# AI-Unicamp/GestureDiffusion

Hardware: AMD Instinct MI355X
Metric: denoised motion frames/sec (1000-step p_sample_loop, B=64, T=196, d=512) (higher is better)
Workload: dtype f32; 1 GPU; BASELINE config 2: MDM_Old (V1 encoder-only topology) J=263 d=512 ff=1024 L=8 H=4, 1000-step p_sample_loop, batch 64/GPU x 196 frames, random weights, in-kernel Philox noise; global_batch=64, frames=196, parallelism=dp1 (independent samples, end-of-loop gather), step=one denoising step (forward + fused sampler update) over the rank's batch

## Files before the change

gesturediffusion_amd/_lib.py:

```python
import ctypes as C
import os

_HERE = os.path.dirname(os.path.abspath(__file__))
LIB_PATH = os.environ.get("GDX_LIBGDX") or os.path.join(_HERE, "csrc", "libgdx.so")

GDX_ARCH_MDM_OLD, GDX_ARCH_MDM = 1, 2
GDX_COND, GDX_UNCOND, GDX_CFG = 0, 1, 2
GDX_SAMPLER_P, GDX_SAMPLER_DDIM = 0, 1
GDX_ROW_PAD = 256

EXPORTS = [
    "gdx_create", "gdx_destroy", "gdx_last_error", "gdx_set_weight", "gdx_weights_ready", "gdx_prepare",
    "gdx_set_condition", "gdx_forward", "gdx_set_keep_taps", "gdx_get_tap", "gdx_sampler_update", "gdx_q_sample",
    "gdx_randn", "gdx_sample_loop", "gdx_bench_ffn_gemm", "gdx_bench_gemm", "gdx_forward_flops", "gdx_profile_begin", "gdx_profile_end", "gdx_bench_attention",
    "gdx_linear_f16", "gdx_linear_f32", "gdx_bench_gemm_f16", "gdx_attention_f16", "gdx_attention_f32", "gdx_plms_update", "gdx_postprocess", "gdx_q_sample_t", "gdx_masked_l2", "gdx_set_graph_replay", "gdx_mfcc",
    "gdx_set_guards", "gdx_check_guards", "gdx_packed_bytes", "gdx_export_packed", "gdx_import_packed", "gdx_set_test_half_dtype",
    "gdx_set_test_gemmh_tile", "gdx_linear_half", "gdx_layernorm", "gdx_local_attention", "gdx_attention_half",
    "gdx_bpd_terms", "gdx_bpd_loop", "gdx_linear_full", "gdx_plms_step", "gdx_plms_loop",
    "gdx_dpm_step", "gdx_dpm_loop", "gdx_dpm_sde_step", "gdx_dpm_sde_loop",
    "gdx_set_guidance_interval", "gdx_forward_samples", "gdx_set_guidance_rescale", "gdx_cfg_rescale",
    "gdx_transpose_in", "gdx_transpose_out", "gdx_small_linear", "gdx_gather_rows", "gdx_mfcc_project", "gdx_token0",
]
GDX_BPD_CHUNK = 4096
INT64_MIN, INT64_MAX = -2**63, 2**63 - 1


class GdxError(RuntimeError):
    pass


class Config(C.Structure):
    _fields_ = [(n, C.c_int32) for n in ("arch", "njoints", "latent_dim", "ff_size", "num_layers", "num_heads",
                                         "seed_poses", "mfcc_dim", "cl_head", "window", "compute_dtype")]


class UpdateArgs(C.Structure):
    _fields_ = [
        ("kind", C.c_int32), ("batch", C.c_int32), ("njoints", C.c_int32), ("frames", C.c_int32),
        ("coef", C.c_void_p), ("t", C.c_void_p), ("step_index", C.c_int32),
        ("x", C.c_void_p), ("x0_cond", C.c_void_p), ("x0_uncond", C.c_void_p), ("scale", C.c_void_p),
        ("inpaint_mask", C.c_void_p), ("inpaint_motion", C.c_void_p), ("noise", C.c_void_p),
        ("const_noise", C.c_int32), ("philox_seed", C.c_uint64), ("sample_offset", C.c_uint64),
        ("rng_step", C.c_uint32), ("out", C.c_void_p), ("pred_xstart", C.c_void_p),
        ("cond_grad", C.c_void_p), ("cond_coef", C.c_void_p), ("clip_denoised", C.c_int32),
    ]


class PlmsArgs(C.Structure):
    _fields_ = [
        ("kind", C.c_int32), ("batch", C.c_int32), ("per_sample", C.c_int64), ("coef", C.c_void_p), ("t", C.c_void_p),
        ("step_index", C.c_int32), ("x", C.c_void_p), ("pred_xstart", C.c_void_p), ("eps", C.c_void_p * 4),
        ("out", C.c_void_p),
    ]

# ... 108 lines not shown
                       f"(run `python __graft_entry__.py` or `make -C gesturediffusion_amd/csrc`)")
    try:
        import torch
        lib = C.CDLL(LIB_PATH)
    except OSError as e:
        raise GdxError(f"cannot load {LIB_PATH}: {e}") from e
    vp, i32, i64, u64, u32 = C.c_void_p, C.c_int32, C.c_int64, C.c_uint64, C.c_uint32
    lib.gdx_last_error.restype = C.c_char_p
    sigs = {
        "gdx_create": [C.POINTER(Config), C.POINTER(vp)],
        "gdx_destroy": [vp],
        "gdx_set_weight": [vp, C.c_char_p, vp, C.POINTER(i64), i32, vp],
        "gdx_weights_ready": [vp],
        "gdx_prepare": [vp, i32, i32],
        "gdx_set_condition": [vp, vp, vp, vp],
        "gdx_forward": [vp, vp, vp, i32, vp, vp, vp],
        "gdx_set_keep_taps": [vp, i32],
        "gdx_get_tap": [vp, i32, vp, i64, vp],
        "gdx_sampler_update": [C.POINTER(UpdateArgs), vp],
        "gdx_q_sample": [vp, vp, vp, i32, i64, vp, vp],
        "gdx_randn": [vp, i32, i64, u64, u64, u32, vp],
        "gdx_sample_loop": [vp, C.POINTER(LoopArgs), vp],
        "gdx_bench_ffn_gemm": [vp, i32, C.POINTER(C.c_float), vp],
        "gdx_forward_flops": [vp, i32, C.POINTER(C.c_double)],
        "gdx_bench_gemm": [i32, i32, i32, i32, i32, C.POINTER(C.c_float), vp],
        "gdx_bench_attention": [i32, i32, i32, i32, i32, i32, C.POINTER(C.c_float), vp],
        "gdx_linear_f16": [vp, vp, vp, vp, vp, i32, i32, i32, i32, vp],
        "gdx_linear_f32": [vp, vp, vp, vp, vp, i32, i32, i32, i32, i32, i32, i32, vp],
        "gdx_linear_half": [vp, vp, vp, vp, i32, vp, i32, vp, vp, i32, i32, i32, i32, i32, i32, i32, i32, i32, i32,
                            C.POINTER(i32), vp],
        "gdx_linear_full": [vp, vp, vp, vp, i32, vp, i32, vp, i32, i32, i32, i32, i32, i32, i32, i32, i32, i32, i32,
                            C.POINTER(i32), vp],
        "gdx_layernorm": [vp, vp, vp, vp, vp, vp, i32, i32, i32, i32, i32, i32, vp],
        "gdx_local_attention": [vp, vp, vp, vp, vp, i32, i32, i32, i32, i32, i32, i32, C.POINTER(i32), vp],
        "gdx_transpose_in": [vp, vp, i32, i32, i32, i32, i32, i32, i32, vp],
        "gdx_transpose_out": [vp, vp, i32, i32, i32, i32, i32, vp],
        "gdx_small_linear": [vp, i32, vp, i32, vp, vp, i32, i32, i32, i32, i32, i32, vp],
        "gdx_gather_rows": [vp, vp, vp, i32, i32, i32, i32, vp],
        "gdx_mfcc_project": [vp, vp, i32, vp, vp, vp, i32, i32, i32, i32, i32, i32, i32, i32, vp],
        "gdx_token0": [vp, i32, vp, vp, vp, vp, i32, vp, vp, vp, i32, vp, i32, i32, i32, i32, i32, vp],
        "gdx_set_graph_replay": [vp, i32],
        "gdx_mfcc": [vp, i64, i32, i32, i32, i32, i32, i32, C.c_float, vp, vp, vp, vp, vp, vp, vp, vp, vp],
        "gdx_q_sample_t": [vp, vp, vp, vp, i32, i64, vp, vp],
        "gdx_masked_l2": [vp, vp, vp, vp, i32, i32, i32, vp],
        "gdx_postprocess": [vp, vp, vp, vp, vp, i32, i32, i32, vp],
        "gdx_plms_update": [C.POINTER(PlmsArgs), vp],
        "gdx_plms_step": [C.POINTER(PlmsStepArgs), vp],
        "gdx_plms_loop": [vp, C.POINTER(PlmsLoopArgs), vp],
        "gdx_dpm_step": [C.POINTER(DpmStepArgs), vp],
        "gdx_dpm_loop": [vp, C.POINTER(DpmLoopArgs), vp],
        "gdx_dpm_sde_step": [C.POINTER(DpmSdeStepArgs), vp],
        "gdx_dpm_sde_loop": [vp, C.POINTER(DpmSdeLoopArgs), vp],
        "gdx_attention_f16": [vp, vp, i32, i32, i32, i32, vp],
        "gdx_attention_half": [vp, i32, vp, i32, i32, i32, i32, i32, i32, i32, i32, C.POINTER(i32), vp],
        "gdx_attention_f32": [vp, vp, i32, i32, i32, i32, i32, vp],
        "gdx_bench_gemm_f16": [i32, i32, i32, i32, i32, C.POINTER(C.c_float), vp],
        "gdx_set_guards": [vp, i32],
        "gdx_check_guards": [vp, C.POINTER(i64), C.POINTER(i32), vp],
        "gdx_set_test_half_dtype": [i32],
        "gdx_set_test_gemmh_tile": [i32, i32],
        "gdx_packed_bytes": [vp, C.POINTER(i64)],
        "gdx_export_packed": [vp, vp, i64, vp],
        "gdx_import_packed": [vp, vp, i64, vp],
        "gdx_bpd_terms": [C.POINTER(BpdArgs), vp],
        "gdx_bpd_loop": [vp, C.POINTER(BpdLoopArgs), vp],
        "gdx_set_guidance_interval": [vp, i64, i64],
# ... 19 lines not shown
```

gesturediffusion_amd/csrc/gdx_internal.h:

```cpp
#pragma once
#include <hip/hip_runtime.h>
#include <stdint.h>

#include "../../include/gdx.h"

#ifdef GDX_BF16
#define GDX_HNS_BEGIN namespace b16 {
#define GDX_HNS_NAME b16
#else
#define GDX_HNS_BEGIN inline namespace h16 {
#define GDX_HNS_NAME h16
#endif
#define GDX_HNS_END }

namespace gdx {

#ifdef GDX_BF16
typedef __bf16 half_t;
#else
typedef _Float16 half_t;
#endif

constexpr int ROW_PAD = GDX_ROW_PAD;

// ... 37 lines not shown
};

struct GemmHParams {
    const _Float16* A; int lda;
    const _Float16* W; int ldw;
    int a_bytes, w_bytes;
    const float* bias;
    const float* R; int ldr;
    const float* V; int ldv;
    float* C32; int ldc32;
    _Float16* C16; int ldc16;
    int M, N, K, T;
    int rowmap, gelu;
};
hipError_t launch_attention(const float* qkv, float* ctx, int B, int S, int H, int d, hipStream_t s);
inline bool head_dim_supported(int hd) { return hd == 32 || hd == 64 || hd == 96 || hd == 128 || hd == 192 || hd == 256; }
#define GDX_HEAD_DIMS "32, 64, 96, 128, 192 or 256"

bool attention3_supported(int S, int H, int d);
hipError_t launch_attention3(const float* qkv, float* ctx, int B, int S, int H, int d, hipStream_t s, int grid = 0);

#define GDX_HALF_API                                                                                                        \
    bool gemmh_supported(const GemmHParams& p);                                                                             \
    hipError_t launch_gemmh(const GemmHParams& p, hipStream_t s, GemmHCtl* ctl = nullptr);                                  \
     \
    bool attentionh_supported(int S, int H, int d);                                                                         \
                              \
    bool attentionh_multiblock(int hd);                                                                                     \
    hipError_t launch_attentionh(const _Float16* qkv, _Float16* ctx, int B, int S, int H, int d, long qkv_rows, hipStream_t s); \
                                                                           \
    hipError_t launch_attentionh_kernel(const _Float16* qkv, _Float16* ctx, int B, int S, int H, int d, long qkv_rows,     \
                                        int kernel, int grid, int* launched, hipStream_t s,                                \
                                        unsigned long long* stamps = nullptr);                                              \
                             \
    hipError_t launch_layernorm(const float* x, const float* res, const float* gamma, const float* beta, float* out,        \
                                _Float16* out16, int rows, int d, int compact_S, hipStream_t s);                            \
      \
    hipError_t launch_layernorm_f16(const _Float16* x, const _Float16* res, const float* gamma, const float* beta,          \
                                    _Float16* out16, float* out32, int rows, int d, int compact_S, hipStream_t s);          \
    hipError_t launch_transpose_in(const float* x, float* xt, int B, int Bsrc, int J, int T, int ldx, hipStream_t s);       \
    hipError_t launch_transpose_in_f16(const float* x, _Float16* xt, int B, int Bsrc, int J, int T, int ldx, hipStream_t s); \
    hipError_t launch_transpose_out(const float* yt, float* y, int B, int J, int T, int ldy, hipStream_t s);                \
                         \
    hipError_t launch_small_linear(const float* A, int lda, const float* W, int ldw, const float* bias, float* out, int ldo, \
                                   int M, int N, int K, int act, hipStream_t s);                                            \
                                                    \
    hipError_t launch_gather_rows(const float* table, const int64_t* idx, float* out, int M, int d, int max_rows, hipStream_t s); \
     \
    hipError_t launch_mfcc_project(const float* mfcc, const float* W, int ldw, const float* bias, const float* pe, float* out, \
                                   int B, int Bsrc, int C, int T, int d, int rps, int off, hipStream_t s);                  \
                                                    \
    hipError_t launch_token0(const float* temb, int tstride, const float* seed_emb, const float* pe0, float* enc,           \
                             _Float16* enc16, const float* c2t, const float* c2_seed, float* c2, const int* state, int B,   \
                             int Bsrc, int S, int d, hipStream_t s);                                                        \
                                           \
    hipError_t launch_local_attention(const float* xseq, const float* cosT, const float* sinT, float* enc, _Float16* enc16, \
                                      int B, int T, int d, int heads, int window, hipStream_t s);                           \
                                     \
    bool local_attention_mfma_supported(int d, int heads, int window);                                                      \
                                                                                       \
    hipError_t launch_convert_f16(const float* src, _Float16* dst, int64_t n, hipStream_t s);                               \
    hipError_t launch_convert_f32(const _Float16* src, float* dst, int64_t n, hipStream_t s);                               \
       \
    bool local_attention_f16_supported(int d, int heads, int window);                                                       \
    hipError_t launch_local_attention_f16(const _Float16* xseq, const float* cosT, const float* sinT, _Float16* enc16,      \
                                          float* enc32, int B, int T, int d, int heads, int window, hipStream_t s);         \
         \
    hipError_t launch_mfcc_frames(const float* x, long n, float* frames, int numframes, int frame_len, int frame_step, int ldf, \
                                  float preemph, hipStream_t s);                                                            \
// ... 39 lines not shown
```

gesturediffusion_amd/csrc/misc.hip:

```cpp
#include "gdx_internal.h"
#include "gdx_device.h"

namespace gdx {
GDX_HNS_BEGIN

__device__ __forceinline__ float wave_sum(float v) {
#pragma unroll
    for (int o = 32; o > 0; o >>= 1) v += __shfl_xor(v, o);
    return v;
}

template <int VPL>
__global__ __launch_bounds__(256) void layernorm_vec_kernel(const float* __restrict__ x, const float* __restrict__ res,
                                                             const float* __restrict__ g,
                                                             const float* __restrict__ bta, float* __restrict__ out,
                                                             half_t* __restrict__ out16, int rows, int d,
                                                             int compact_S) {
    const int row = blockIdx.x * 4 + (threadIdx.x >> 6);
    const int lane = threadIdx.x & 63;
    if (row >= rows) return;
    long orow = row;
    if (compact_S > 0) {
        const int b = row / compact_S;
        if (row - b * compact_S == 0) return;
        orow = row - b - 1;
    }
    const f32x4* xp = reinterpret_cast<const f32x4*>(x + (long)row * d);
    const f32x4* rp = reinterpret_cast<const f32x4*>(res + (long)row * d);
    f32x4 v[VPL];
    float s = 0.0f;
#pragma unroll
    for (int i = 0; i < VPL; ++i) {
        v[i] = xp[lane + 64 * i];
        if (res) v[i] += rp[lane + 64 * i];
        s += (v[i][0] + v[i][1]) + (v[i][2] + v[i][3]);
    }
    const float mean = wave_sum(s) / (float)d;
    float q = 0.0f;
#pragma unroll
    for (int i = 0; i < VPL; ++i)
#pragma unroll
        for (int e = 0; e < 4; ++e) {
            const float c = v[i][e] - mean;
            q += c * c;
        }
    const float rstd = 1.0f / sqrtf(wave_sum(q) / (float)d + 1e-5f);
    f32x4* op = reinterpret_cast<f32x4*>(out + orow * d);
    f16x4* hp = reinterpret_cast<f16x4*>(out16 + orow * d);
    const f32x4* gp = reinterpret_cast<const f32x4*>(g);
    const f32x4* bp = reinterpret_cast<const f32x4*>(bta);
#pragma unroll
    for (int i = 0; i < VPL; ++i) {
        const f32x4 gg = gp[lane + 64 * i], bb = bp[lane + 64 * i];
        f32x4 r;
#pragma unroll
        for (int e = 0; e < 4; ++e) r[e] = (v[i][e] - mean) * rstd * gg[e] + bb[e];
        if (out) op[lane + 64 * i] = r;
        if (out16) hp[lane + 64 * i] = f16x4{(half_t)r[0], (half_t)r[1], (half_t)r[2], (half_t)r[3]};
    }
}

__global__ __launch_bounds__(256) void layernorm_gen_kernel(const float* __restrict__ x, const float* __restrict__ res,
                                                             const float* __restrict__ g,
                                                             const float* __restrict__ bta, float* __restrict__ out,
                                                             half_t* __restrict__ out16, int rows, int d,
                                                             int compact_S) {
    const int row = blockIdx.x * 4 + (threadIdx.x >> 6);
    const int lane = threadIdx.x & 63;
    if (row >= rows) return;
    long orow = row;
    if (compact_S > 0) {
        const int b = row / compact_S;
        if (row - b * compact_S == 0) return;
        orow = row - b - 1;
    }
    const float* xp = x + (long)row * d;
    const float* rp = res + (long)row * d;
    float s = 0.0f;
    for (int e = lane; e < d; e += 64) s += res ? xp[e] + rp[e] : xp[e];
    const float mean = wave_sum(s) / (float)d;
    float q = 0.0f;
    for (int e = lane; e < d; e += 64) {
        const float c = (res ? xp[e] + rp[e] : xp[e]) - mean;
        q += c * c;
    }
    const float rstd = 1.0f / sqrtf(wave_sum(q) / (float)d + 1e-5f);
    for (int e = lane; e < d; e += 64) {
        const float r = ((res ? xp[e] + rp[e] : xp[e]) - mean) * rstd * g[e] + bta[e];
        if (out) out[orow * d + e] = r;
        if (out16) out16[orow * d + e] = (half_t)r;
    }
}

hipError_t launch_layernorm(const float* x, const float* res, const float* gamma, const float* beta, float* out,
                            _Float16* out16_, int rows, int d, int compact_S, hipStream_t s) {
    half_t* out16 = reinterpret_cast<half_t*>(out16_);
    const dim3 grid((rows + 3) / 4), block(256);
    if (d == 512)
        hipLaunchKernelGGL(layernorm_vec_kernel<2>, grid, block, 0, s, x, res, gamma, beta, out, out16, rows, d, compact_S);
    else if (d == 1024)
        hipLaunchKernelGGL(layernorm_vec_kernel<4>, grid, block, 0, s, x, res, gamma, beta, out, out16, rows, d, compact_S);
    else if (d == 256)
        hipLaunchKernelGGL(layernorm_vec_kernel<1>, grid, block, 0, s, x, res, gamma, beta, out, out16, rows, d, compact_S);
    else
        hipLaunchKernelGGL(layernorm_gen_kernel, grid, block, 0, s, x, res, gamma, beta, out, out16, rows, d, compact_S);
    return hipGetLastError();
}

template <int NV>
__global__ __launch_bounds__(256) void layernorm_h_vec_kernel(const half_t* __restrict__ x, const half_t* __restrict__ res,
                                                               const float* __restrict__ g, const float* __restrict__ bta,
                                                               half_t* __restrict__ out16, float* __restrict__ out32,
                                                               int rows, int d, int compact_S) {
    const int row = blockIdx.x * 4 + (threadIdx.x >> 6);
    const int lane = threadIdx.x & 63;
    if (row >= rows) return;
    long orow = row;
    if (compact_S > 0) {
        const int b = row / compact_S;
        if (row - b * compact_S == 0) return;
        orow = row - b - 1;
    }
    const f16x8* xp = reinterpret_cast<const f16x8*>(x + (long)row * d);
    const f16x8* rp = reinterpret_cast<const f16x8*>(res + (long)row * d);
    float v[NV][8];
    float s = 0.0f;
#pragma unroll
    for (int i = 0; i < NV; ++i) {
        const f16x8 a = xp[lane + 64 * i];
        f16x8 r = f16x8{0, 0, 0, 0, 0, 0, 0, 0};
        if (res) r = rp[lane + 64 * i];
#pragma unroll
        for (int e = 0; e < 8; ++e) {
            v[i][e] = (float)a[e] + (float)r[e];
            s += v[i][e];
        }
    }
    const float mean = wave_sum(s) / (float)d;
// ... 732 lines not shown
```

gesturediffusion_amd/csrc/sampler.hip:

```cpp
#include <string>

#include "gdx_internal.h"
#include "gdx_device.h"
#include "../../include/gdx.h"

#pragma clang fp contract(off)

namespace gdx {


struct Philox {
    static constexpr uint32_t M0 = 0xD2511F53u, M1 = 0xCD9E8D57u, W0 = 0x9E3779B9u, W1 = 0xBB67AE85u;
    __device__ static void run(uint32_t c[4], uint32_t k0, uint32_t k1) {
#pragma unroll
        for (int r = 0; r < 10; ++r) {
            const uint32_t hi0 = __umulhi(M0, c[0]), lo0 = M0 * c[0];
            const uint32_t hi1 = __umulhi(M1, c[2]), lo1 = M1 * c[2];
            const uint32_t n0 = hi1 ^ c[1] ^ k0, n2 = hi0 ^ c[3] ^ k1;
            c[0] = n0; c[1] = lo1; c[2] = n2; c[3] = lo0;
            k0 += W0; k1 += W1;
        }
    }
};

// ... 150 lines not shown
    uint64_t seed, sample_offset;
    uint32_t rng_step;
    const int* state;
    long noise_stride;
    const float* grad;
    const float* gcoef;
};

template <bool VEC>
__global__ __launch_bounds__(256) void update_kernel(const UpdateDev a) {
    const long gid = (long)blockIdx.x * 256 + threadIdx.x;
    if (gid >= a.s.groups * a.batch) return;
    const Group g = group_of<VEC>(gid, a.s.groups, a.s.per_sample);
    const long idx = a.state ? a.state[0] : coef_row(a.s, g.b);
    const float* c = a.s.coef + idx * 8;
    const uint32_t rng_step = a.state ? (uint32_t)a.state[1] + 1u : a.rng_step;
    const float* noise = a.noise && a.state ? a.noise + (long)a.state[1] * a.noise_stride : a.noise;

    const f32x4 x = load4<VEC>(a.s.x, g.e0, g.nval);
    const f32x4 x0 = pred_xstart4<VEC>(a.s, g);
    const f32x4 z = noise ? load4<VEC>(noise, a.const_noise ? 4L * g.grp : g.e0, g.nval)
                          : philox_normal4(a.seed, a.const_noise ? 0ull : a.sample_offset + (uint64_t)g.b, rng_step, g.grp);
    const bool cond = a.grad != nullptr;
    const f32x4 grad = cond ? load4<VEC>(a.grad, g.e0, g.nval) : f32x4{0.f, 0.f, 0.f, 0.f};
    const float s1m = cond && a.kind != GDX_SAMPLER_P ? a.gcoef[idx] : 0.0f;
    f32x4 r;
#pragma unroll
    for (int i = 0; i < 4; ++i) r[i] = update_value(a.kind, c, x[i], x0[i], z[i], cond, grad[i], s1m);
    store4<VEC>(a.s.out, g.e0, g.nval, r);
    if (a.s.pred) store4<VEC>(a.s.pred, g.e0, g.nval, x0);
}

__global__ __launch_bounds__(256) void update_tm_kernel(const UpdateTmDev a) {
    const int jq_n = (a.J + 3) / 4, tq_n = a.T / 4;
    const long gid = (long)blockIdx.x * 256 + threadIdx.x;
    if (gid >= (long)a.B * tq_n * jq_n) return;
    const int jq = gid % jq_n;
    const long bt = gid / jq_n;
    const int tq = bt % tq_n, b = bt / tq_n;
    const int j0 = 4 * jq, t0 = 4 * tq;
    const float* c = a.coef + (long)a.step_index * 8;
    const long row0 = (long)b * a.T + t0;
    const long urow = (long)a.B * a.T;
    const bool both = a.scale || a.mirror;
    f32x4 x[4], x0[4];
#pragma unroll
    for (int tt = 0; tt < 4; ++tt) {
        x[tt] = *reinterpret_cast<const f32x4*>(a.xt + (row0 + tt) * a.ldx + j0);
        x0[tt] = *reinterpret_cast<const f32x4*>(a.x0t + (row0 + tt) * a.ldo + j0);
    }
    if (a.scale) {
        const float sc = a.scale[b];
#pragma unroll
        for (int tt = 0; tt < 4; ++tt) {
            const f32x4 u = *reinterpret_cast<const f32x4*>(a.x0t + (urow + row0 + tt) * a.ldo + j0);
#pragma unroll
            for (int jj = 0; jj < 4; ++jj) x0[tt][jj] = cfg_blend(x0[tt][jj], u[jj], sc);
        }
    }
    if (a.clip) {
#pragma unroll
        for (int tt = 0; tt < 4; ++tt)
#pragma unroll
            for (int jj = 0; jj < 4; ++jj) x0[tt][jj] = clamp1(x0[tt][jj]);
    }
    const uint64_t sample = a.const_noise ? 0ull : a.sample_offset + (uint64_t)b;
    f32x4 r[4];
#pragma unroll
    for (int jj = 0; jj < 4; ++jj) {
        const int j = j0 + jj;
        if (j < a.J) {
            const f32x4 z = a.noise ? *reinterpret_cast<const f32x4*>(a.noise + ((long)(a.const_noise ? 0 : b) * a.J + j) * a.T + t0)
                                    : philox_normal4(a.seed, sample, a.rng_step, (uint32_t)(j * tq_n + tq));
#pragma unroll
            for (int tt = 0; tt < 4; ++tt) r[tt][jj] = update_value(a.kind, c, x[tt][jj], x0[tt][jj], z[tt]);
        } else {
#pragma unroll
            for (int tt = 0; tt < 4; ++tt) r[tt][jj] = 0.0f;
        }
    }
#pragma unroll
    for (int tt = 0; tt < 4; ++tt) {
        *reinterpret_cast<f32x4*>(a.xt + (row0 + tt) * a.ldx + j0) = r[tt];
        if (both) *reinterpret_cast<f32x4*>(a.xt + (urow + row0 + tt) * a.ldx + j0) = r[tt];
    }
    if (a.xt16) {
        typedef _Float16 h4 __attribute__((ext_vector_type(4)));
        typedef __bf16 b4 __attribute__((ext_vector_type(4)));
#pragma unroll
        for (int tt = 0; tt < 4; ++tt) {
            const long o0 = (row0 + tt) * a.ldx + j0, o1 = o0 + urow * a.ldx;
            if (a.half_dtype == GDX_DTYPE_BF16) {
                const b4 v = b4{(__bf16)r[tt][0], (__bf16)r[tt][1], (__bf16)r[tt][2], (__bf16)r[tt][3]};
                *reinterpret_cast<b4*>((__bf16*)a.xt16 + o0) = v;
                if (both) *reinterpret_cast<b4*>((__bf16*)a.xt16 + o1) = v;
            } else {
                const h4 v = h4{(_Float16)r[tt][0], (_Float16)r[tt][1], (_Float16)r[tt][2], (_Float16)r[tt][3]};
                *reinterpret_cast<h4*>((_Float16*)a.xt16 + o0) = v;
                if (both) *reinterpret_cast<h4*>((_Float16*)a.xt16 + o1) = v;
            }
        }
    }
    if (a.out_pose) {
#pragma unroll
        for (int jj = 0; jj < 4; ++jj)
            if (j0 + jj < a.J)
                *reinterpret_cast<f32x4*>(a.out_pose + ((long)b * a.J + j0 + jj) * a.T + t0) = f32x4{r[0][jj], r[1][jj], r[2][jj], r[3][jj]};
    }
}

__global__ void q_sample_kernel(const float* __restrict__ xs, const float* __restrict__ nz, const float* coef,
                                int idx, const int64_t* __restrict__ t, long per_sample, long n, float* __restrict__ out) {
    const long i = (long)blockIdx.x * blockDim.x + threadIdx.x;
    if (i >= n) return;
    const long row = t ? (long)t[i / per_sample] : (long)idx;
    const float a = coef[row * 8 + 5], b = coef[row * 8 + 6];
    out[i] = q_sample_value(a, b, xs[i], nz[i]);
}

__global__ void plms_kernel(int kind, const float* __restrict__ coef, const int64_t* __restrict__ t, int step_index,
                            const float* __restrict__ x, const float* __restrict__ x0, const float* __restrict__ e0,
                            const float* __restrict__ e1, const float* __restrict__ e2, const float* __restrict__ e3,
                            float* __restrict__ out, long per_sample, long total) {
    const long i = (long)blockIdx.x * blockDim.x + threadIdx.x;
    if (i >= total) return;
    const long idx = t ? (long)t[i / per_sample] : (long)step_index;
    const float* c = coef + idx * 8;
    if (kind == 0) out[i] = eps_from_xstart(c[0], c[1], x[i], x0[i]);
    else if (kind == 6) out[i] = ddim_mean(c[2], c[3], x0[i], e0[i]);
    else if (kind == 7) out[i] = cond_score_xstart(c[0], c[1], e1[idx], x[i], x0[i], e0[i]);
    else if (kind == 8) out[i] = xstart_from_eps(c[0], c[1], x[i], x0[i]);
    else {
        const float v1 = kind != 1 ? e1[i] : 0.f, v2 = kind == 3 || kind == 4 ? e2[i] : 0.f, v3 = kind == 4 ? e3[i] : 0.f;
        out[i] = plms_tail(c, x[i], plms_combine(kind, e0[i], v1, v2, v3), x0[i]);
    }
}

struct PlmsStepDev {
    StepSrc s;
    const int64_t* t_eps;
    int step_index_eps;
// ... 387 lines not shown
static gdx::StepSrc step_src(const A* a, float* pred) {
    gdx::StepSrc s;
    s.per_sample = (long)a->njoints * a->frames;
    s.groups = (s.per_sample + 3) / 4;
    s.coef = a->coef; s.t = a->t; s.step_index = a->step_index;
    s.x = a->x; s.x0c = a->x0_cond; s.x0u = a->x0_uncond; s.scale = a->scale;
    s.mask = a->inpaint_mask; s.motion = a->inpaint_motion; s.clip = a->clip_denoised;
    s.out = a->out; s.pred = pred;
    return s;
}

template <typename A, typename Entry, typename Hist>
static int step_begin(const char* who, const A* a, float* A::*pred, Entry entry_check, Hist hist_check, gdx::StepSrc& s, dim3& grid) {
    if (!a || !a->coef || !a->x || !a->x0_cond || !a->out) return refuse(who, "null argument");
    if (const char* m = entry_check()) return refuse(who, m);
    if (a->batch < 0 || a->njoints < 0 || a->frames < 0 || a->batch > 65535) return refuse(who, "bad shape");
    if (a->x0_uncond && !a->scale) return refuse(who, "CFG needs scale");
    if (a->inpaint_mask && !a->inpaint_motion) return refuse(who, "mask without motion");
    if (const char* m = hist_check()) return refuse(who, m);
    s = step_src(a, a->*pred);
    if (a->batch == 0 || s.per_sample == 0) return 1;
    grid = dim3((unsigned)((s.groups + 255) / 256), (unsigned)a->batch);
    return 0;
}

static int sampler_update_impl(const gdx_update_args_t* a, const int* state, long noise_stride, void* stream);

int gdx_sampler_update_tm_(const gdx::UpdateTmDev& d, void* stream) {
    using namespace gdx;
    const int jpad = (d.J + 3) / 4 * 4;
    if (!d.coef || !d.xt || !d.x0t || d.T % 4 || d.ldx % 4 || d.ldo % 4 || d.ldx < jpad || d.ldo < jpad)
        return gdx_set_error_("gdx_sampler_update_tm_: bad argument");
    if (d.noise && ((uintptr_t)d.noise & 15)) return gdx_set_error_("gdx_sampler_update_tm_: noise tape not 16-byte aligned");
    const long total = (long)d.B * (d.T / 4) * (jpad / 4);
    if (total == 0) return 0;
    hipLaunchKernelGGL(update_tm_kernel, dim3((total + 255) / 256), dim3(256), 0, (hipStream_t)stream, d);
    return launch_status("gdx_sampler_update_tm_: launch failed");
}

extern "C" int gdx_sampler_update(const gdx_update_args_t* a, void* stream) {
    return sampler_update_impl(a, nullptr, 0, stream);
}

int gdx_sampler_update_state_(const gdx_update_args_t* a, const int* state, long noise_stride, void* stream) {
    return sampler_update_impl(a, state, noise_stride, stream);
}

static int sampler_update_impl(const gdx_update_args_t* a, const int* state, long noise_stride, void* stream) {
    using namespace gdx;
    if (!a || !a->coef || !a->x || !a->x0_cond || !a->out) return gdx_set_error_("gdx_sampler_update: null argument");
    if (a->x0_uncond && !a->scale) return gdx_set_error_("gdx_sampler_update: CFG needs scale");
    if (a->inpaint_mask && !a->inpaint_motion) return gdx_set_error_("gdx_sampler_update: mask without motion");
    UpdateDev d;
    d.s = step_src(a, a->pred_xstart);
    d.kind = a->kind; d.batch = a->batch;
    d.noise = a->noise; d.const_noise = a->const_noise;
    d.seed = a->philox_seed; d.sample_offset = a->sample_offset; d.rng_step = a->rng_step;
    d.state = state; d.noise_stride = noise_stride;
    d.grad = a->cond_grad; d.gcoef = a->cond_coef;
    if (d.grad && a->kind != GDX_SAMPLER_P && !d.gcoef) return gdx_set_error_("gdx_sampler_update: cond_grad needs cond_coef for DDIM");
    const long total = d.s.groups * d.batch;
    if (total == 0) return 0;
    const dim3 grid((total + 255) / 256), block(256);
    if (vec_ok(d.s, d.noise, d.grad))
        hipLaunchKernelGGL(update_kernel<true>, grid, block, 0, (hipStream_t)stream, d);
    else
        hipLaunchKernelGGL(update_kernel<false>, grid, block, 0, (hipStream_t)stream, d);
// ... 234 lines not shown
```

gesturediffusion_amd/csrc/testapi.hip:

```cpp
#include "gdx_host.h"

#include <cstdio>
#include <cstdlib>

using namespace gdx;

static bool t_bf16 = false;
static int t_gemmh_mb = -1, t_gemmh_nbw = -1;

namespace {

struct Scratch {
    const std::string who;
    const hipStream_t s;
    const bool bf;
    std::vector<void*> pool;
    Scratch(const char* who, hipStream_t s, bool bf = false) : who(who), s(s), bf(bf) {}
    ~Scratch() {
        (void)hipStreamSynchronize(s);
        free_pool(pool);
    }
    template <class T>
    int alloc(T** p, size_t bytes) { return dev_alloc(pool, (void**)p, bytes); }
    int to_half(_Float16** h, const float* src, int64_t n) {
// ... 175 lines not shown
        return -1;
    GemmHParams p{a16, K, w16, K, (int)((size_t)M * K * 2), (int)((size_t)npad * K * 2), bias, R, ldr, V, ldv,
                  C32, N, c16, N, M, N, K, T, rowmap, gelu};
    GemmHCtl ctl;
    ctl.mb = force_mb; ctl.nbw = force_nbw;
    const hipError_t e = HFN(bf, launch_gemmh, p, s, &ctl);
    if (launched) {
        const GemmHLaunched& l = ctl.ran;
        launched[0] = l.mb; launched[1] = l.nbw; launched[2] = l.main_rows; launched[3] = l.tail_mb; launched[4] = l.tail_nbw;
    }
    if (e != hipSuccess) return fail(std::string("launch_gemmh: ") + hipGetErrorString(e));
    return C16 ? sc.widen(c16, C16, (int64_t)c_rows * N) : 0;
}

extern "C" int gdx_linear_half(const float* A, const float* W, const float* bias, const float* R, int32_t ldr, const float* V,
                               int32_t ldv, float* C32, float* C16, int32_t c_rows, int32_t M, int32_t N, int32_t K, int32_t T,
                               int32_t rowmap, int32_t gelu, int32_t dtype, int32_t tile_mb, int32_t tile_nbw,
                               int32_t* launched, void* stream) {
    if ((dtype != GDX_DTYPE_F16 && dtype != GDX_DTYPE_BF16) || tile_mb < 0 || tile_nbw < 0 || (tile_mb == 0) != (tile_nbw == 0))
        return fail("gdx_linear_half: bad argument");
    return linear_half("gdx_linear_half", A, W, bias, R, ldr, V, ldv, C32, C16, c_rows, M, N, K, T, rowmap, gelu,
                       dtype == GDX_DTYPE_BF16, tile_mb, tile_nbw, launched, (hipStream_t)stream);
}

extern "C" int gdx_linear_f16(const float* A, const float* W, const float* bias, float* C32, float* C16, int32_t M,
                              int32_t N, int32_t K, int32_t gelu, void* stream) {
    return linear_half("gdx_linear_f16", A, W, bias, nullptr, 0, nullptr, 0, C32, C16, M, M, N, K, 1, 0, gelu, t_bf16,
                       t_gemmh_mb, t_gemmh_nbw, nullptr, (hipStream_t)stream);
}

extern "C" int gdx_layernorm(const float* x, const float* res, const float* gamma, const float* beta, float* out32,
                             float* out16, int32_t out_rows, int32_t rows, int32_t d, int32_t compact_S, int32_t half_input,
                             int32_t dtype, void* stream) {
    const long need = compact_S > 0 ? (long)rows - (rows + compact_S - 1) / compact_S : rows;
    if (!x || !gamma || !beta || (!out32 && !out16) || rows <= 0 || d <= 0 || d % 32 || d > 2048 || compact_S < 0 ||
        out_rows < need || (dtype != GDX_DTYPE_F32 && dtype != GDX_DTYPE_F16 && dtype != GDX_DTYPE_BF16) ||
        (dtype == GDX_DTYPE_F32 && (half_input || out16)) || (half_input && !out16))
        return fail("gdx_layernorm: bad argument");
    hipStream_t s = (hipStream_t)stream;
    const bool bf = dtype == GDX_DTYPE_BF16;
    const int64_t n_in = (int64_t)rows * d, n_out = (int64_t)out_rows * d;
    _Float16 *x16 = nullptr, *r16 = nullptr, *o16 = nullptr;
    Scratch sc("gdx_layernorm", s, bf);
    if ((half_input && (sc.to_half(&x16, x, n_in) || (res && sc.to_half(&r16, res, n_in)))) ||
        (out16 && sc.to_half(&o16, out16, n_out)))
        return -1;
    const hipError_t e = half_input ? HFN(bf, launch_layernorm_f16, x16, r16, gamma, beta, o16, out32, rows, d, compact_S, s)
                                    : HFN(bf, launch_layernorm, x, res, gamma, beta, out32, o16, rows, d, compact_S, s);
    if (e != hipSuccess) return fail(std::string("launch_layernorm: ") + hipGetErrorString(e));
    return out16 ? sc.widen(o16, out16, n_out) : 0;
}

extern "C" int gdx_local_attention(const float* xseq, const float* cosT, const float* sinT, float* enc, float* enc16,
                                   int32_t enc_rows, int32_t B, int32_t T, int32_t d, int32_t heads, int32_t window,
                                   int32_t dtype, int32_t* kernel, void* stream) {
    const bool dt_ok = dtype == GDX_DTYPE_F32 || dtype == GDX_DTYPE_F16 || dtype == GDX_DTYPE_BF16;
    if (!xseq || !cosT || !sinT || !dt_ok || B <= 0 || T <= 0 || heads <= 0 || d <= 0 || d % heads || (d / heads) % 2 ||
        window <= 0 || T % window || enc_rows < (long)B * (T + 1) || (dtype == GDX_DTYPE_F32 && enc16))
        return fail("gdx_local_attention: bad argument");
    const bool half = local_attention_half(dtype, d, heads, window);
    if (!half && !enc) return fail("gdx_local_attention: the fp32 kernel needs enc");
    if (half && !enc16) return fail("gdx_local_attention: the 16-bit kernel needs enc16");
    hipStream_t s = (hipStream_t)stream;
    const int64_t n_in = (int64_t)B * T * d, n_out = (int64_t)enc_rows * d;
    _Float16 *x16 = nullptr, *e16 = nullptr;
    Scratch sc("gdx_local_attention", s, dtype == GDX_DTYPE_BF16);
    if (kernel) *kernel = half ? 2 : local_attention_mfma_supported(d, heads, window) ? 1 : 0;
    if ((half && sc.to_half(&x16, xseq, n_in)) || (enc16 && sc.to_half(&e16, enc16, n_out))) return -1;
    const hipError_t e = launch_local_attention_any(dtype, xseq, x16, cosT, sinT, enc, e16, B, T, d, heads, window, s);
    if (e != hipSuccess) return fail(std::string("launch_local_attention: ") + hipGetErrorString(e));
    return enc16 ? sc.widen(e16, enc16, n_out) : 0;
}

static bool dtype_known(int dtype) { return dtype == GDX_DTYPE_F32 || dtype == GDX_DTYPE_F16 || dtype == GDX_DTYPE_BF16; }

extern "C" int gdx_transpose_in(const float* x, float* xt, int32_t xt_rows, int32_t B, int32_t Bsrc, int32_t J, int32_t T,
                                int32_t ldx, int32_t dtype, void* stream) {
    if (!x || !xt || B <= 0 || B > 65535 || Bsrc <= 0 || Bsrc > B || J <= 0 || T <= 0) return fail("gdx_transpose_in: bad argument");
    if (!dtype_known(dtype)) return fail("gdx_transpose_in: unknown dtype");
    if (ldx < J) return fail("gdx_transpose_in: ldx below J");
    if (xt_rows < (long)B * T) return fail("gdx_transpose_in: xt_rows below B*T");
// ... 241 lines not shown
```

include/gdx.h:

```cpp
#ifndef GDX_H
#define GDX_H

#include <stdint.h>

#ifdef __cplusplus
extern "C" {
#endif

typedef struct gdx_model* gdx_handle_t;

#define GDX_ROW_PAD 256

enum { GDX_ARCH_MDM_OLD = 1,
       GDX_ARCH_MDM = 2 };

enum { GDX_COND = 0,
       GDX_UNCOND = 1,
       GDX_CFG = 2 };

enum { GDX_DTYPE_F32 = 0,
       GDX_DTYPE_F16 = 1,
       GDX_DTYPE_BF16 = 2 };

enum { GDX_SAMPLER_P = 0,
// ... 301 lines not shown
    const float* coef;
    const int64_t* timestep_map;
    float* x;
    const float* scale;
    const uint8_t* inpaint_mask;
    const float* inpaint_motion;
    int32_t clip_denoised;
    int32_t run_steps;
    int32_t k_base;
    float* hist;
    const float* noise_tape;
    uint64_t philox_seed;
    uint64_t sample_offset;
} gdx_dpm_sde_loop_args_t;
int gdx_dpm_sde_loop(gdx_handle_t h, const gdx_dpm_sde_loop_args_t* a, void* stream);

int gdx_set_graph_replay(gdx_handle_t h, int32_t on);

int gdx_bench_ffn_gemm(gdx_handle_t h, int32_t iters, float* avg_us, void* stream);
int gdx_profile_begin(gdx_handle_t h, int32_t max_launches);
int gdx_profile_end(gdx_handle_t h, float* avg_us, int32_t* launches);
int gdx_bench_gemm(int32_t M, int32_t N, int32_t K, int32_t epi, int32_t iters, float* avg_us, void* stream);
int gdx_bench_attention(int32_t B, int32_t S, int32_t H, int32_t d, int32_t version, int32_t iters,
                        float* avg_us, void* stream);
int gdx_linear_f16(const float* A, const float* W, const float* bias, float* C32, float* C16,
                   int32_t M, int32_t N, int32_t K, int32_t gelu, void* stream);
int gdx_linear_half(const float* A, const float* W, const float* bias, const float* R, int32_t ldr, const float* V,
                    int32_t ldv, float* C32, float* C16, int32_t c_rows, int32_t M, int32_t N, int32_t K, int32_t T,
                    int32_t rowmap, int32_t gelu, int32_t dtype, int32_t tile_mb, int32_t tile_nbw, int32_t* launched,
                    void* stream);
int gdx_layernorm(const float* x, const float* res, const float* gamma, const float* beta, float* out32, float* out16,
                  int32_t out_rows, int32_t rows, int32_t d, int32_t compact_S, int32_t half_input, int32_t dtype,
                  void* stream);
int gdx_local_attention(const float* xseq, const float* cosT, const float* sinT, float* enc, float* enc16, int32_t enc_rows,
                        int32_t B, int32_t T, int32_t d, int32_t heads, int32_t window, int32_t dtype, int32_t* kernel,
                        void* stream);
int gdx_transpose_in(const float* x, float* xt, int32_t xt_rows, int32_t B, int32_t Bsrc, int32_t J, int32_t T, int32_t ldx,
                     int32_t dtype, void* stream);
int gdx_transpose_out(const float* yt, float* y, int32_t y_rows, int32_t B, int32_t J, int32_t T, int32_t ldy, void* stream);
int gdx_small_linear(const float* A, int32_t lda, const float* W, int32_t ldw, const float* bias, float* out, int32_t out_rows,
                     int32_t ldo, int32_t M, int32_t N, int32_t K, int32_t act, void* stream);
int gdx_gather_rows(const float* table, const int64_t* idx, float* out, int32_t out_rows, int32_t M, int32_t d,
                    int32_t max_rows, void* stream);
int gdx_mfcc_project(const float* mfcc, const float* W, int32_t ldw, const float* bias, const float* pe, float* out,
                     int32_t out_rows, int32_t B, int32_t Bsrc, int32_t C, int32_t T, int32_t d, int32_t rps, int32_t off,
                     void* stream);
int gdx_token0(const float* temb, int32_t tstride, const float* seed_emb, const float* pe0, float* enc, float* enc16,
               int32_t enc_rows, const float* c2t, const float* c2_seed, float* c2, int32_t c2_rows, const int32_t* state,
               int32_t B, int32_t Bsrc, int32_t S, int32_t d, int32_t dtype, void* stream);
int gdx_attention_f16(const float* qkv, float* ctx, int32_t B, int32_t S, int32_t H, int32_t d, void* stream);
int gdx_attention_half(const float* qkv, int32_t qkv_rows, float* ctx, int32_t ctx_rows, int32_t B, int32_t S, int32_t H,
                       int32_t d, int32_t dtype, int32_t kernel, int32_t grid, int32_t* launched, void* stream);
int gdx_set_test_half_dtype(int32_t dtype);
int gdx_set_test_gemmh_tile(int32_t mb, int32_t nbw);
int gdx_attention_f32(const float* qkv, float* ctx, int32_t B, int32_t S, int32_t H, int32_t d, int32_t version,
                      void* stream);
int gdx_linear_f32(const float* A, const float* W, const float* bias, const float* R, float* C, int32_t M, int32_t N,
                   int32_t K, int32_t epi, int32_t tile_mb, int32_t tile_nbw, int32_t tile_bk, void* stream);
int gdx_linear_full(const float* A, const float* W, const float* bias, const float* R, int32_t ldr, const float* V,
                    int32_t ldv, float* C, int32_t c_rows, int32_t M, int32_t N, int32_t K, int32_t T, int32_t rowmap,
                    int32_t gelu, int32_t kernel, int32_t tile_mb, int32_t tile_nbw, int32_t tile_bk, int32_t* launched,
                    void* stream);
int gdx_bench_gemm_f16(int32_t M, int32_t N, int32_t K, int32_t gelu, int32_t iters, float* avg_us,
                       void* stream);
int gdx_forward_flops(gdx_handle_t h, int32_t mode, double* flops);

// ... 5 lines not shown
```

Baseline: 3092 frames/s.

## Make layernorm grid-stride with row prefetch; scalarize sampler update layout

The vector layernorm kernel becomes a persistent grid-stride kernel. The grid is sized to resident occupancy across the CUs, gamma and beta are loaded once per wave, and the next row is prefetched while the current row is reduced. The residual path becomes a template parameter and compact-row indexing is inverted to iterate over output rows. Separately, the transposed sampler update kernel now uses one thread per joint instead of a 4x4 joint tile, trading vector loads for coalesced scalar accesses across joints. This adds a test entry point with a forced grid.

```diff
diff --git a/gesturediffusion_amd/_lib.py b/gesturediffusion_amd/_lib.py
--- a/gesturediffusion_amd/_lib.py
+++ b/gesturediffusion_amd/_lib.py
@@ -20,6 +20,7 @@
     "gdx_dpm_step", "gdx_dpm_loop", "gdx_dpm_sde_step", "gdx_dpm_sde_loop",
     "gdx_set_guidance_interval", "gdx_forward_samples", "gdx_set_guidance_rescale", "gdx_cfg_rescale",
     "gdx_transpose_in", "gdx_transpose_out", "gdx_small_linear", "gdx_gather_rows", "gdx_mfcc_project", "gdx_token0",
+    "gdx_layernorm_grid",
 ]
 GDX_BPD_CHUNK = 4096
 INT64_MIN, INT64_MAX = -2**63, 2**63 - 1
@@ -194,6 +195,7 @@
         "gdx_linear_full": [vp, vp, vp, vp, i32, vp, i32, vp, i32, i32, i32, i32, i32, i32, i32, i32, i32, i32, i32,
                             C.POINTER(i32), vp],
         "gdx_layernorm": [vp, vp, vp, vp, vp, vp, i32, i32, i32, i32, i32, i32, vp],
+        "gdx_layernorm_grid": [vp, vp, vp, vp, vp, vp, i32, i32, i32, i32, i32, i32, i32, vp],
         "gdx_local_attention": [vp, vp, vp, vp, vp, i32, i32, i32, i32, i32, i32, i32, C.POINTER(i32), vp],
         "gdx_transpose_in": [vp, vp, i32, i32, i32, i32, i32, i32, i32, vp],
         "gdx_transpose_out": [vp, vp, i32, i32, i32, i32, i32, vp],
diff --git a/gesturediffusion_amd/csrc/gdx_internal.h b/gesturediffusion_amd/csrc/gdx_internal.h
--- a/gesturediffusion_amd/csrc/gdx_internal.h
+++ b/gesturediffusion_amd/csrc/gdx_internal.h
@@ -93,9 +93,9 @@
     hipError_t launch_attentionh_kernel(const _Float16* qkv, _Float16* ctx, int B, int S, int H, int d, long qkv_rows,     \
                                         int kernel, int grid, int* launched, hipStream_t s,                                \
                                         unsigned long long* stamps = nullptr);                                              \
-                             \
+                    \
     hipError_t launch_layernorm(const float* x, const float* res, const float* gamma, const float* beta, float* out,        \
-                                _Float16* out16, int rows, int d, int compact_S, hipStream_t s);                            \
+                                _Float16* out16, int rows, int d, int compact_S, hipStream_t s, int grid = 0);              \
       \
     hipError_t launch_layernorm_f16(const _Float16* x, const _Float16* res, const float* gamma, const float* beta,          \
                                     _Float16* out16, float* out32, int rows, int d, int compact_S, hipStream_t s);          \
diff --git a/gesturediffusion_amd/csrc/misc.hip b/gesturediffusion_amd/csrc/misc.hip
--- a/gesturediffusion_amd/csrc/misc.hip
+++ b/gesturediffusion_amd/csrc/misc.hip
@@ -2,6 +2,7 @@
 #include "gdx_device.h"
 
 namespace gdx {
+int gemm2_num_cus();
 GDX_HNS_BEGIN
 
 __device__ __forceinline__ float wave_sum(float v) {
@@ -10,54 +11,69 @@
     return v;
 }
 
-template <int VPL>
+template <int VPL, bool RES>
 __global__ __launch_bounds__(256) void layernorm_vec_kernel(const float* __restrict__ x, const float* __restrict__ res,
                                                              const float* __restrict__ g,
                                                              const float* __restrict__ bta, float* __restrict__ out,
                                                              half_t* __restrict__ out16, int rows, int d,
                                                              int compact_S) {
-    const int row = blockIdx.x * 4 + (threadIdx.x >> 6);
+    const int nwaves = gridDim.x * 4;
     const int lane = threadIdx.x & 63;
-    if (row >= rows) return;
-    long orow = row;
-    if (compact_S > 0) {
-        const int b = row / compact_S;
-        if (row - b * compact_S == 0) return;
-        orow = row - b - 1;
-    }
-    const f32x4* xp = reinterpret_cast<const f32x4*>(x + (long)row * d);
-    const f32x4* rp = reinterpret_cast<const f32x4*>(res + (long)row * d);
-    f32x4 v[VPL];
-    float s = 0.0f;
+    const int nout = compact_S > 0 ? rows - (rows + compact_S - 1) / compact_S : rows;
+    int o = blockIdx.x * 4 + (threadIdx.x >> 6);
+    if (o >= nout) return;
+    f32x4 nx[VPL], nr[VPL];
+    auto fetch = [&](int orow) {
+        const long r = compact_S > 0 ? orow + orow / (compact_S - 1) + 1 : orow;
+        const f32x4* xp = reinterpret_cast<const f32x4*>(x + r * d);
+        const f32x4* rp = reinterpret_cast<const f32x4*>(res + r * d);
+#pragma unroll
+        for (int i = 0; i < VPL; ++i) {
+            nx[i] = xp[lane + 64 * i];
+            if (RES) nr[i] = rp[lane + 64 * i];
+        }
+    };
+    f32x4 gg[VPL], bb[VPL];
 #pragma unroll
     for (int i = 0; i < VPL; ++i) {
-        v[i] = xp[lane + 64 * i];
-        if (res) v[i] += rp[lane + 64 * i];
-        s += (v[i][0] + v[i][1]) + (v[i][2] + v[i][3]);
-    }
-    const float mean = wave_sum(s) / (float)d;
-    float q = 0.0f;
-#pragma unroll
-    for (int i = 0; i < VPL; ++i)
-#pragma unroll
-        for (int e = 0; e < 4; ++e) {
-            const float c = v[i][e] - mean;
-            q += c * c;
-        }
-    const float rstd = 1.0f / sqrtf(wave_sum(q) / (float)d + 1e-5f);
-    f32x4* op = reinterpret_cast<f32x4*>(out + orow * d);
-    f16x4* hp = reinterpret_cast<f16x4*>(out16 + orow * d);
-    const f32x4* gp = reinterpret_cast<const f32x4*>(g);
-    const f32x4* bp = reinterpret_cast<const f32x4*>(bta);
-#pragma unroll
-    for (int i = 0; i < VPL; ++i) {
-        const f32x4 gg = gp[lane + 64 * i], bb = bp[lane + 64 * i];
-        f32x4 r;
-#pragma unroll
-        for (int e = 0; e < 4; ++e) r[e] = (v[i][e] - mean) * rstd * gg[e] + bb[e];
-        if (out) op[lane + 64 * i] = r;
-        if (out16) hp[lane + 64 * i] = f16x4{(half_t)r[0], (half_t)r[1], (half_t)r[2], (half_t)r[3]};
-    }
+        gg[i] = reinterpret_cast<const f32x4*>(g)[lane + 64 * i];
+        bb[i] = reinterpret_cast<const f32x4*>(bta)[lane + 64 * i];
+    }
+    fetch(o);
+    auto one_row = [&](long orow, bool more) {
+        f32x4 v[VPL];
+        float s = 0.0f;
+#pragma unroll
+        for (int i = 0; i < VPL; ++i) {
+            v[i] = nx[i];
+            if (RES) v[i] += nr[i];
+            s += (v[i][0] + v[i][1]) + (v[i][2] + v[i][3]);
+        }
+        if (more) fetch((int)orow + nwaves);
+        const float mean = wave_sum(s) / (float)d;
+        float q = 0.0f;
+#pragma unroll
+        for (int i = 0; i < VPL; ++i)
+#pragma unroll
+            for (int e = 0; e < 4; ++e) {
+                const float c = v[i][e] - mean;
+                q += c * c;
+            }
+        const float rstd = 1.0f / sqrtf(wave_sum(q) / (float)d + 1e-5f);
+        f32x4* op = reinterpret_cast<f32x4*>(out + orow * d);
+        f16x4* hp = reinterpret_cast<f16x4*>(out16 + orow * d);
+#pragma unroll
+        for (int i = 0; i < VPL; ++i) {
+            f32x4 r4;
+#pragma unroll
+            for (int e = 0; e < 4; ++e) r4[e] = (v[i][e] - mean) * rstd * gg[i][e] + bb[i][e];
+            if (out) op[lane + 64 * i] = r4;
+            if (out16) hp[lane + 64 * i] = f16x4{(half_t)r4[0], (half_t)r4[1], (half_t)r4[2], (half_t)r4[3]};
+        }
+    };
+#pragma unroll 1
+    for (; o + nwaves < nout; o += nwaves) one_row(o, true);
+    one_row(o, false);
 }
 
 __global__ __launch_bounds__(256) void layernorm_gen_kernel(const float* __restrict__ x, const float* __restrict__ res,
@@ -92,18 +108,40 @@
     }
 }
 
+template <int VPL, bool RES>
+static void launch_ln_inst(const float* x, const float* res, const float* gamma, const float* beta, float* out, half_t* out16,
+                           int rows, int d, int compact_S, hipStream_t s, int grid_force) {
+    static int resident = 0;
+    auto kernel = layernorm_vec_kernel<VPL, RES>;
+    const int nout = compact_S > 0 ? rows - (rows + compact_S - 1) / compact_S : rows;
+    if (nout <= 0) return;
+    if (!resident) {
+        int per_cu = 0;
+        if (hipOccupancyMaxActiveBlocksPerMultiprocessor(&per_cu, kernel, 256, 0) != hipSuccess || per_cu <= 0) per_cu = 4;
+        resident = per_cu * gemm2_num_cus();
+    }
+    const int all = (nout + 3) / 4, want = grid_force > 0 ? grid_force : all <= 4 * resident ? resident : all;
+    hipLaunchKernelGGL(kernel, dim3(want < all ? want : all), dim3(256), 0, s, x, res, gamma, beta, out, out16, rows, d, compact_S);
+}
+template <int VPL>
+static void launch_ln_vec(const float* x, const float* res, const float* gamma, const float* beta, float* out, half_t* out16,
+                          int rows, int d, int compact_S, hipStream_t s, int grid_force) {
+    if (res) launch_ln_inst<VPL, true>(x, res, gamma, beta, out, out16, rows, d, compact_S, s, grid_force);
+    else launch_ln_inst<VPL, false>(x, res, gamma, beta, out, out16, rows, d, compact_S, s, grid_force);
+}
+
 hipError_t launch_layernorm(const float* x, const float* res, const float* gamma, const float* beta, float* out,
-                            _Float16* out16_, int rows, int d, int compact_S, hipStream_t s) {
+                            _Float16* out16_, int rows, int d, int compact_S, hipStream_t s, int grid_force) {
     half_t* out16 = reinterpret_cast<half_t*>(out16_);
-    const dim3 grid((rows + 3) / 4), block(256);
+    const dim3 block(256);
     if (d == 512)
-        hipLaunchKernelGGL(layernorm_vec_kernel<2>, grid, block, 0, s, x, res, gamma, beta, out, out16, rows, d, compact_S);
+        launch_ln_vec<2>(x, res, gamma, beta, out, out16, rows, d, compact_S, s, grid_force);
     else if (d == 1024)
-        hipLaunchKernelGGL(layernorm_vec_kernel<4>, grid, block, 0, s, x, res, gamma, beta, out, out16, rows, d, compact_S);
+        launch_ln_vec<4>(x, res, gamma, beta, out, out16, rows, d, compact_S, s, grid_force);
     else if (d == 256)
-        hipLaunchKernelGGL(layernorm_vec_kernel<1>, grid, block, 0, s, x, res, gamma, beta, out, out16, rows, d, compact_S);
+        launch_ln_vec<1>(x, res, gamma, beta, out, out16, rows, d, compact_S, s, grid_force);
     else
-        hipLaunchKernelGGL(layernorm_gen_kernel, grid, block, 0, s, x, res, gamma, beta, out, out16, rows, d, compact_S);
+        hipLaunchKernelGGL(layernorm_gen_kernel, dim3((rows + 3) / 4), block, 0, s, x, res, gamma, beta, out, out16, rows, d, compact_S);
     return hipGetLastError();
 }
 
diff --git a/gesturediffusion_amd/csrc/sampler.hip b/gesturediffusion_amd/csrc/sampler.hip
--- a/gesturediffusion_amd/csrc/sampler.hip
+++ b/gesturediffusion_amd/csrc/sampler.hip
@@ -206,81 +206,61 @@
 }
 
 __global__ __launch_bounds__(256) void update_tm_kernel(const UpdateTmDev a) {
-    const int jq_n = (a.J + 3) / 4, tq_n = a.T / 4;
+    const int jpad = (a.J + 3) / 4 * 4, tq_n = a.T / 4;
     const long gid = (long)blockIdx.x * 256 + threadIdx.x;
-    if (gid >= (long)a.B * tq_n * jq_n) return;
-    const int jq = gid % jq_n;
-    const long bt = gid / jq_n;
+    if (gid >= (long)a.B * tq_n * jpad) return;
+    const int j = gid % jpad;
+    const long bt = gid / jpad;
     const int tq = bt % tq_n, b = bt / tq_n;
-    const int j0 = 4 * jq, t0 = 4 * tq;
+    const int t0 = 4 * tq;
     const float* c = a.coef + (long)a.step_index * 8;
     const long row0 = (long)b * a.T + t0;
     const long urow = (long)a.B * a.T;
     const bool both = a.scale || a.mirror;
-    f32x4 x[4], x0[4];
+    f32x4 r = f32x4{0.f, 0.f, 0.f, 0.f};
+    if (j < a.J) {
+        f32x4 x, x0;
+#pragma unroll
+        for (int tt = 0; tt < 4; ++tt) {
+            x[tt] = a.xt[(row0 + tt) * a.ldx + j];
+            x0[tt] = a.x0t[(row0 + tt) * a.ldo + j];
+        }
+        if (a.scale) {
+            const float sc = a.scale[b];
+#pragma unroll
+            for (int tt = 0; tt < 4; ++tt) x0[tt] = cfg_blend(x0[tt], a.x0t[(urow + row0 + tt) * a.ldo + j], sc);
+        }
+        if (a.clip) {
+#pragma unroll
+            for (int tt = 0; tt < 4; ++tt) x0[tt] = clamp1(x0[tt]);
+        }
+        const uint64_t sample = a.const_noise ? 0ull : a.sample_offset + (uint64_t)b;
+        const f32x4 z = a.noise ? *reinterpret_cast<const f32x4*>(a.noise + ((long)(a.const_noise ? 0 : b) * a.J + j) * a.T + t0)
+                                : philox_normal4(a.seed, sample, a.rng_step, (uint32_t)(j * tq_n + tq));
+#pragma unroll
+        for (int tt = 0; tt < 4; ++tt) r[tt] = update_value(a.kind, c, x[tt], x0[tt], z[tt]);
+    }
 #pragma unroll
     for (int tt = 0; tt < 4; ++tt) {
-        x[tt] = *reinterpret_cast<const f32x4*>(a.xt + (row0 + tt) * a.ldx + j0);
-        x0[tt] = *reinterpret_cast<const f32x4*>(a.x0t + (row0 + tt) * a.ldo + j0);
-    }
-    if (a.scale) {
-        const float sc = a.scale[b];
+        a.xt[(row0 + tt) * a.ldx + j] = r[tt];
+        if (both) a.xt[(urow + row0 + tt) * a.ldx + j] = r[tt];
+    }
+    if (a.xt16) {
 #pragma unroll
         for (int tt = 0; tt < 4; ++tt) {
-            const f32x4 u = *reinterpret_cast<const f32x4*>(a.x0t + (urow + row0 + tt) * a.ldo + j0);
-#pragma unroll
-            for (int jj = 0; jj < 4; ++jj) x0[tt][jj] = cfg_blend(x0[tt][jj], u[jj], sc);
-        }
-    }
-    if (a.clip) {
-#pragma unroll
-        for (int tt = 0; tt < 4; ++tt)
-#pragma unroll
-            for (int jj = 0; jj < 4; ++jj) x0[tt][jj] = clamp1(x0[tt][jj]);
-    }
-    const uint64_t sample = a.const_noise ? 0ull : a.sample_offset + (uint64_t)b;
-    f32x4 r[4];
-#pragma unroll
-    for (int jj = 0; jj < 4; ++jj) {
-        const int j = j0 + jj;
-        if (j < a.J) {
-            const f32x4 z = a.noise ? *reinterpret_cast<const f32x4*>(a.noise + ((long)(a.const_noise ? 0 : b) * a.J + j) * a.T + t0)
-                                    : philox_normal4(a.seed, sample, a.rng_step, (uint32_t)(j * tq_n + tq));
-#pragma unroll
-            for (int tt = 0; tt < 4; ++tt) r[tt][jj] = update_value(a.kind, c, x[tt][jj], x0[tt][jj], z[tt]);
-        } else {
-#pragma unroll
-            for (int tt = 0; tt < 4; ++tt) r[tt][jj] = 0.0f;
-        }
-    }
-#pragma unroll
-    for (int tt = 0; tt < 4; ++tt) {
-        *reinterpret_cast<f32x4*>(a.xt + (row0 + tt) * a.ldx + j0) = r[tt];
-        if (both) *reinterpret_cast<f32x4*>(a.xt + (urow + row0 + tt) * a.ldx + j0) = r[tt];
-    }
-    if (a.xt16) {
-        typedef _Float16 h4 __attribute__((ext_vector_type(4)));
-        typedef __bf16 b4 __attribute__((ext_vector_type(4)));
-#pragma unroll
-        for (int tt = 0; tt < 4; ++tt) {
-            const long o0 = (row0 + tt) * a.ldx + j0, o1 = o0 + urow * a.ldx;
+            const long o0 = (row0 + tt) * a.ldx + j, o1 = o0 + urow * a.ldx;
             if (a.half_dtype == GDX_DTYPE_BF16) {
-                const b4 v = b4{(__bf16)r[tt][0], (__bf16)r[tt][1], (__bf16)r[tt][2], (__bf16)r[tt][3]};
-                *reinterpret_cast<b4*>((__bf16*)a.xt16 + o0) = v;
-                if (both) *reinterpret_cast<b4*>((__bf16*)a.xt16 + o1) = v;
+                const __bf16 v = (__bf16)r[tt];
+                ((__bf16*)a.xt16)[o0] = v;
+                if (both) ((__bf16*)a.xt16)[o1] = v;
             } else {
-                const h4 v = h4{(_Float16)r[tt][0], (_Float16)r[tt][1], (_Float16)r[tt][2], (_Float16)r[tt][3]};
-                *reinterpret_cast<h4*>((_Float16*)a.xt16 + o0) = v;
-                if (both) *reinterpret_cast<h4*>((_Float16*)a.xt16 + o1) = v;
+                const _Float16 v = (_Float16)r[tt];
+                ((_Float16*)a.xt16)[o0] = v;
+                if (both) ((_Float16*)a.xt16)[o1] = v;
             }
         }
     }
-    if (a.out_pose) {
-#pragma unroll
-        for (int jj = 0; jj < 4; ++jj)
-            if (j0 + jj < a.J)
-                *reinterpret_cast<f32x4*>(a.out_pose + ((long)b * a.J + j0 + jj) * a.T + t0) = f32x4{r[0][jj], r[1][jj], r[2][jj], r[3][jj]};
-    }
+    if (a.out_pose && j < a.J) *reinterpret_cast<f32x4*>(a.out_pose + ((long)b * a.J + j) * a.T + t0) = r;
 }
 
 __global__ void q_sample_kernel(const float* __restrict__ xs, const float* __restrict__ nz, const float* coef,
@@ -734,7 +714,7 @@
     if (!d.coef || !d.xt || !d.x0t || d.T % 4 || d.ldx % 4 || d.ldo % 4 || d.ldx < jpad || d.ldo < jpad)
         return gdx_set_error_("gdx_sampler_update_tm_: bad argument");
     if (d.noise && ((uintptr_t)d.noise & 15)) return gdx_set_error_("gdx_sampler_update_tm_: noise tape not 16-byte aligned");
-    const long total = (long)d.B * (d.T / 4) * (jpad / 4);
+    const long total = (long)d.B * (d.T / 4) * jpad;
     if (total == 0) return 0;
     hipLaunchKernelGGL(update_tm_kernel, dim3((total + 255) / 256), dim3(256), 0, (hipStream_t)stream, d);
     return launch_status("gdx_sampler_update_tm_: launch failed");
diff --git a/gesturediffusion_amd/csrc/testapi.hip b/gesturediffusion_amd/csrc/testapi.hip
--- a/gesturediffusion_amd/csrc/testapi.hip
+++ b/gesturediffusion_amd/csrc/testapi.hip
@@ -231,10 +231,16 @@
 extern "C" int gdx_layernorm(const float* x, const float* res, const float* gamma, const float* beta, float* out32,
                              float* out16, int32_t out_rows, int32_t rows, int32_t d, int32_t compact_S, int32_t half_input,
                              int32_t dtype, void* stream) {
+    return gdx_layernorm_grid(x, res, gamma, beta, out32, out16, out_rows, rows, d, compact_S, half_input, dtype, 0, stream);
+}
+
+extern "C" int gdx_layernorm_grid(const float* x, const float* res, const float* gamma, const float* beta, float* out32,
+                                  float* out16, int32_t out_rows, int32_t rows, int32_t d, int32_t compact_S,
+                                  int32_t half_input, int32_t dtype, int32_t grid, void* stream) {
     const long need = compact_S > 0 ? (long)rows - (rows + compact_S - 1) / compact_S : rows;
     if (!x || !gamma || !beta || (!out32 && !out16) || rows <= 0 || d <= 0 || d % 32 || d > 2048 || compact_S < 0 ||
         out_rows < need || (dtype != GDX_DTYPE_F32 && dtype != GDX_DTYPE_F16 && dtype != GDX_DTYPE_BF16) ||
-        (dtype == GDX_DTYPE_F32 && (half_input || out16)) || (half_input && !out16))
+        (dtype == GDX_DTYPE_F32 && (half_input || out16)) || (half_input && !out16) || grid < 0 || (grid && half_input))
         return fail("gdx_layernorm: bad argument");
     hipStream_t s = (hipStream_t)stream;
     const bool bf = dtype == GDX_DTYPE_BF16;
@@ -245,7 +251,7 @@
         (out16 && sc.to_half(&o16, out16, n_out)))
         return -1;
     const hipError_t e = half_input ? HFN(bf, launch_layernorm_f16, x16, r16, gamma, beta, o16, out32, rows, d, compact_S, s)
-                                    : HFN(bf, launch_layernorm, x, res, gamma, beta, out32, o16, rows, d, compact_S, s);
+                                    : HFN(bf, launch_layernorm, x, res, gamma, beta, out32, o16, rows, d, compact_S, s, grid);
     if (e != hipSuccess) return fail(std::string("launch_layernorm: ") + hipGetErrorString(e));
     return out16 ? sc.widen(o16, out16, n_out) : 0;
 }
diff --git a/include/gdx.h b/include/gdx.h
--- a/include/gdx.h
+++ b/include/gdx.h
@@ -357,6 +357,9 @@
 int gdx_layernorm(const float* x, const float* res, const float* gamma, const float* beta, float* out32, float* out16,
                   int32_t out_rows, int32_t rows, int32_t d, int32_t compact_S, int32_t half_input, int32_t dtype,
                   void* stream);
+int gdx_layernorm_grid(const float* x, const float* res, const float* gamma, const float* beta, float* out32, float* out16,
+                       int32_t out_rows, int32_t rows, int32_t d, int32_t compact_S, int32_t half_input, int32_t dtype,
+                       int32_t grid, void* stream);
 int gdx_local_attention(const float* xseq, const float* cosT, const float* sinT, float* enc, float* enc16, int32_t enc_rows,
                         int32_t B, int32_t T, int32_t d, int32_t heads, int32_t window, int32_t dtype, int32_t* kernel,
                         void* stream);
```

Measured after the change: 3102 frames/s (median of 6 runs). Within noise of the previous version (+0.3%).
